# ExistentialRobotics/CORSAIR

Hardware: AMD Instinct MI355X
Metric: end-to-end queries/sec (embed+retrieve+register), Scan2CAD chair (higher is better)
Workload: dtype f32 sparse conv + embedding / f64 RANSAC, k-NN, Chamfer, top-k / f16 MFMA bounds and shortlists (survivors recounted in f64)

## Files before the change

### corsair_amd/csrc/ransac.hip

```cpp
#include <math.h>

#include <algorithm>
#include <atomic>
#include <vector>

#include "common.h"
#include "horn.h"

namespace cs {

using f32x16 = __attribute__((ext_vector_type(16))) float;
using f32x2 = __attribute__((ext_vector_type(2))) float;

struct RansacProb {
  int64_t off;
  int32_t m;
  int32_t est_k;
  int32_t best_cnt;
  int32_t best_itr;
  unsigned long long best_err;
  int32_t done;
  int32_t iters;
  int32_t n_cand;
  int32_t chunk_max;
  double best_T[12];
};

__device__ __forceinline__ RansacProb prob_view(const RansacProb* probs, int p) {
  RansacProb v = {};
  v.off = probs[p].off;
  v.m = probs[p].m;
  v.est_k = __atomic_load_n(&probs[p].est_k, __ATOMIC_RELAXED);
  v.done = __atomic_load_n(&probs[p].done, __ATOMIC_RELAXED);
  return v;
}

__host__ __device__ static inline uint32_t rng_index(uint64_t seed, uint64_t itr, uint64_t j,
                                                     uint32_t m) {
  return (uint32_t)(((rng_u64(seed, itr, j) >> 32) * (uint64_t)m) >> 32);
}

__global__ void k_ransac_pack(const float* __restrict__ src, const float* __restrict__ tgt,
                              int64_t n, float* __restrict__ pk, float4* __restrict__ pair32) {
  int64_t i = blockIdx.x * (int64_t)blockDim.x + threadIdx.x;
  if (i >= n) return;
  pair32[2 * i + 0] = make_float4(src[3 * i + 0], src[3 * i + 1], src[3 * i + 2], tgt[3 * i + 0]);
  pair32[2 * i + 1] = make_float4(tgt[3 * i + 1], tgt[3 * i + 2], 0.f, 0.f);
  pk[0 * n + i] = src[3 * i + 0];
  pk[1 * n + i] = src[3 * i + 1];
  pk[2 * n + i] = src[3 * i + 2];
  pk[3 * n + i] = tgt[3 * i + 0];
  pk[4 * n + i] = tgt[3 * i + 1];
  pk[5 * n + i] = tgt[3 * i + 2];
}

constexpr int XCD_SLOTS = 64;
struct XcdTab {
  int32_t v[8 * XCD_SLOTS];
};
__device__ __forceinline__ int xcd_problem(const int32_t* __restrict__ xcd_ptr, const XcdTab& tab, int i) {
  return xcd_ptr ? xcd_ptr[i] : tab.v[i];
}

__device__ __forceinline__ void pf_emit_row(const RansacProb& pr, int p, int h, int bmax, const double (&R)[3][3], double (&t)[3],
                                            const unsigned* __restrict__ stat, const double* __restrict__ sums, double thr2,
                                            double tcap, _Float16* __restrict__ A16, float* __restrict__ c_h);

template <int RN>
__global__ __launch_bounds__(256) void k_ransac_hyp(const RansacProb* probs,
                                                    const float4* __restrict__ pair32, int it0,
                                                    int bcount, int bmax, int ransac_n,
                                                    uint64_t seed,
                                                    const int32_t* __restrict__ xcd_prob, const XcdTab xcd_tab,
                                                    int slots, int tiles, int force_jacobi,
                                                    double* __restrict__ hyp,
                                                    const unsigned* __restrict__ pf_stat, const double* __restrict__ pf_sums,
                                                    double thr2, double tcap, _Float16* __restrict__ A16,
                                                    float* __restrict__ c_h, int32_t* __restrict__ cnt_zero) {
  const int xcd = blockIdx.x & 7;
  const int item = blockIdx.x >> 3;
  const int slot = item / tiles;
  const int p = xcd_problem(xcd_prob, xcd_tab, xcd * slots + slot);
  if (p < 0) return;
  const int h = (item - slot * tiles) * blockDim.x + threadIdx.x;
  if (h >= bcount) return;
  if (cnt_zero) cnt_zero[(int64_t)p * bmax + h] = 0;
  const RansacProb pr = prob_view(probs, p);
  const int itr = it0 + h;
  if (pr.done || itr >= pr.est_k) return;
  const uint32_t m = (uint32_t)pr.m;
  double cs_[3] = {0, 0, 0}, ct_[3] = {0, 0, 0};
  double S[3][3] = {{0, 0, 0}, {0, 0, 0}, {0, 0, 0}};
  if (RN > 0) {
    float4 pa[RN > 0 ? RN : 1];
    float2 pb[RN > 0 ? RN : 1];
#pragma unroll
    for (int j = 0; j < RN; ++j) {
      const int64_t i = pr.off + rng_index(seed, (uint64_t)itr, (uint64_t)j, m);
      const float4 a = pair32[2 * i], b = pair32[2 * i + 1];
      pa[j] = a;
      pb[j] = make_float2(b.x, b.y);
      cs_[0] += (double)a.x;
      cs_[1] += (double)a.y;
      cs_[2] += (double)a.z;
      ct_[0] += (double)a.w;
      ct_[1] += (double)b.x;
      ct_[2] += (double)b.y;
    }
    const double dn = (double)RN;
#pragma unroll
    for (int a = 0; a < 3; ++a) {
      cs_[a] = cs_[a] / dn;
      ct_[a] = ct_[a] / dn;
    }
#pragma unroll
    for (int j = 0; j < RN; ++j) {
      const double ds[3] = {(double)pa[j].x - cs_[0], (double)pa[j].y - cs_[1], (double)pa[j].z - cs_[2]};
      const double dt[3] = {(double)pa[j].w - ct_[0], (double)pb[j].x - ct_[1], (double)pb[j].y - ct_[2]};
#pragma unroll
      for (int a = 0; a < 3; ++a)
#pragma unroll
        for (int b = 0; b < 3; ++b) S[a][b] = fma(ds[a], dt[b], S[a][b]);
    }
  } else {
    for (int j = 0; j < ransac_n; ++j) {
      const int64_t i = pr.off + rng_index(seed, (uint64_t)itr, (uint64_t)j, m);
      const float4 a = pair32[2 * i], b = pair32[2 * i + 1];
      cs_[0] += (double)a.x;
      cs_[1] += (double)a.y;
      cs_[2] += (double)a.z;
      ct_[0] += (double)a.w;
      ct_[1] += (double)b.x;
      ct_[2] += (double)b.y;
    }
    const double dn = (double)ransac_n;
#pragma unroll
    for (int a = 0; a < 3; ++a) {
      cs_[a] = cs_[a] / dn;
      ct_[a] = ct_[a] / dn;
    }
    for (int j = 0; j < ransac_n; ++j) {
      const int64_t i = pr.off + rng_index(seed, (uint64_t)itr, (uint64_t)j, m);
      const float4 a = pair32[2 * i], b = pair32[2 * i + 1];
      const double ds[3] = {(double)a.x - cs_[0], (double)a.y - cs_[1], (double)a.z - cs_[2]};
      const double dt[3] = {(double)a.w - ct_[0], (double)b.x - ct_[1], (double)b.y - ct_[2]};
#pragma unroll
      for (int a = 0; a < 3; ++a)
#pragma unroll
        for (int b = 0; b < 3; ++b) S[a][b] = fma(ds[a], dt[b], S[a][b]);
    }
  }
  double N[4][4], V[4][4];
  N[0][0] = S[0][0] + S[1][1] + S[2][2];
  N[0][1] = S[1][2] - S[2][1];
  N[0][2] = S[2][0] - S[0][2];
  N[0][3] = S[0][1] - S[1][0];
  N[1][1] = S[0][0] - S[1][1] - S[2][2];
  N[1][2] = S[0][1] + S[1][0];
  N[1][3] = S[2][0] + S[0][2];
  N[2][2] = -S[0][0] + S[1][1] - S[2][2];
  N[2][3] = S[1][2] + S[2][1];
  N[3][3] = -S[0][0] - S[1][1] + S[2][2];
  N[1][0] = N[0][1];
  N[2][0] = N[0][2];
  N[3][0] = N[0][3];
  N[2][1] = N[1][2];
  N[3][1] = N[1][3];
  N[3][2] = N[2][3];
  double qv[4];
  if (force_jacobi || !horn_qcp(S, N, qv)) {
    jacobi4(N, V);
    double best = N[0][0];
    qv[0] = V[0][0]; qv[1] = V[1][0]; qv[2] = V[2][0]; qv[3] = V[3][0];
#pragma unroll
    for (int c = 1; c < 4; ++c) {
      if (N[c][c] > best) {
        best = N[c][c];
        qv[0] = V[0][c];
        qv[1] = V[1][c];
        qv[2] = V[2][c];
        qv[3] = V[3][c];
      }
    }
  }
  double qw = qv[0], qx = qv[1], qy = qv[2], qz = qv[3];
  const double qn = sqrt(qw * qw + qx * qx + qy * qy + qz * qz);
  qw = qw / qn;
  qx = qx / qn;
  qy = qy / qn;
  qz = qz / qn;
  double R[3][3];
  R[0][0] = 1.0 - 2.0 * (qy * qy + qz * qz);
  R[0][1] = 2.0 * (qx * qy - qw * qz);
// ... 107 lines not shown
    else
      atomicAdd(&res_cnt[(int64_t)p * bmax + hsel], cnt);
  }
}

template <bool LIST, int HPW = RC_HYP>
__global__ __launch_bounds__(256) void k_ransac_count(const RansacProb* __restrict__ probs,
                                                      const float* __restrict__ pk, int64_t total,
                                                      const double* __restrict__ hyp, int it0,
                                                      int bcount, int bmax, int splits, double thr2,
                                                      int32_t* __restrict__ res_cnt,
                                                      const int32_t* __restrict__ hlist,
                                                      const int32_t* __restrict__ n_surv) {
  __shared__ __attribute__((aligned(16))) double lds[2][RC_CHUNK][6];
  const int p = blockIdx.y;
  const int tile0 = blockIdx.x / splits;
  const int split = blockIdx.x - tile0 * splits;
  if (LIST) {
    const int nlist = n_surv[p];
    const int tstride = gridDim.x / splits;
    for (int tile = tile0; tile * RC_HYP < nlist; tile += tstride) {
      ransac_count_tile<LIST, HPW>(lds, p, tile, split, probs, pk, total, hyp, it0, bcount, bmax, splits, thr2,
                                   res_cnt, hlist, n_surv);
      __syncthreads();
    }
  } else {
    ransac_count_tile<LIST, HPW>(lds, p, tile0, split, probs, pk, total, hyp, it0, bcount, bmax, splits, thr2,
                                 res_cnt, hlist, n_surv);
  }
}

using f16x8 = __attribute__((ext_vector_type(8))) _Float16;
constexpr int PF_K = 16;
constexpr int PF_PITCH = 40;
constexpr int PF_PITCH1 = 24;
__host__ __device__ constexpr int pf_pitch(int nm) { return nm == 2 ? PF_PITCH : PF_PITCH1; }
constexpr int PF_ROWS = 192;
constexpr int PF_NG = 2;
constexpr int PF_HYP = 4 * 32 * PF_NG;
constexpr int PF_STAT = 17;
constexpr float PF_SMAX = 128.0f;

__device__ __forceinline__ _Float16 f16_of(double v) { return (_Float16)(float)v; }

__device__ __forceinline__ void split16(double v, _Float16* hi, _Float16* lo) {
  const _Float16 h = f16_of(v);
  *hi = h;
  *lo = f16_of(v - (double)h);
}

__host__ __device__ static inline int64_t pf_padded(int64_t m) { return (m + PF_ROWS - 1) / PF_ROWS * PF_ROWS; }

__global__ __launch_bounds__(256) void k_ransac_pair_sums(const RansacProb* __restrict__ probs, const float* __restrict__ src,
                                                          const float* __restrict__ tgt, double* __restrict__ sums) {
  __shared__ double red[4][6];
  const RansacProb pr = probs[blockIdx.x];
  double a[6] = {0, 0, 0, 0, 0, 0};
  for (int j = threadIdx.x; j < pr.m; j += 256) {
    const int64_t i = pr.off + j;
#pragma unroll
    for (int c = 0; c < 3; ++c) {
      a[c] += (double)src[3 * i + c];
      a[3 + c] += (double)tgt[3 * i + c];
    }
  }
#pragma unroll
  for (int c = 0; c < 6; ++c) {
#pragma unroll
    for (int off = 32; off >= 1; off >>= 1) a[c] += __shfl_xor(a[c], off);
    if ((threadIdx.x & 63) == 0) red[threadIdx.x >> 6][c] = a[c];
  }
  __syncthreads();
  if (threadIdx.x < 6) {
    const double sum = (red[0][threadIdx.x] + red[1][threadIdx.x]) + (red[2][threadIdx.x] + red[3][threadIdx.x]);
    const double v = sum / (double)(pr.m > 0 ? pr.m : 1);
    sums[blockIdx.x * 6 + threadIdx.x] = (v == v && fabs(v) < 1.0e30) ? v : 0.0;
  }
}
__device__ __forceinline__ void pf_centre(const double* __restrict__ sums, int p, int m, double (&mu)[6]) {
  (void)m;
#pragma unroll
  for (int c = 0; c < 6; ++c) mu[c] = sums[p * 6 + c];
}

template <int NM>
__global__ __launch_bounds__(256) void k_ransac_pack16(const RansacProb* __restrict__ probs,
                                                       const int64_t* __restrict__ off16,
                                                       const float* __restrict__ src,
                                                       const float* __restrict__ tgt,
                                                       const double* __restrict__ sums,
                                                       _Float16* __restrict__ B16,
                                                       unsigned* __restrict__ stat) {
  __shared__ float red[4][PF_STAT];
  const RansacProb pr = probs[blockIdx.y];
  double mu[6];
  pf_centre(sums, blockIdx.y, pr.m, mu);
  const int mpad = (int)pf_padded(pr.m);
  float mx[PF_STAT];
#pragma unroll
  for (int k = 0; k < PF_STAT; ++k) mx[k] = 0.f;
  for (int j = blockIdx.x * blockDim.x + threadIdx.x; j < mpad; j += gridDim.x * blockDim.x) {
    constexpr int NV = pf_pitch(NM) / 8;
    union {
      _Float16 h[PF_PITCH];
      uint4 v[5];
    } row;
#pragma unroll
    for (int k = 0; k < 5; ++k) row.v[k] = make_uint4(0u, 0u, 0u, 0u);
    if (j < pr.m) {
      const int64_t i = pr.off + j;
      const double sx = src[3 * i] - mu[0], sy = src[3 * i + 1] - mu[1], sz = src[3 * i + 2] - mu[2];
      const double qx = tgt[3 * i] - mu[3], qy = tgt[3 * i + 1] - mu[4], qz = tgt[3 * i + 2] - mu[5];
      const double ss = sx * sx + sy * sy + sz * sz, qq = qx * qx + qy * qy + qz * qz;
      double b[16];
      b[0] = ss + qq;
      b[1] = sx; b[2] = sy; b[3] = sz;
      b[4] = qx * sx; b[5] = qx * sy; b[6] = qx * sz;
      b[7] = qy * sx; b[8] = qy * sy; b[9] = qy * sz;
      b[10] = qz * sx; b[11] = qz * sy; b[12] = qz * sz;
      b[13] = qx; b[14] = qy; b[15] = qz;
      float mag = 1.0000002f * (float)sqrt(fmax(ss, qq));
      const bool ok = mag <= PF_SMAX;
      if (!(mag == mag)) mag = INFINITY;
#pragma unroll
      for (int k = 0; k < 16; ++k) {
        _Float16 hi = (_Float16)0.0f, lo = (_Float16)0.0f;
        if (ok) {
          split16(b[k], &hi, &lo);
          mx[1 + k] = fmaxf(mx[1 + k], __double2float_ru(fabs(b[k])));
        }
        row.h[k] = hi;
        if (NM == 2) row.h[16 + k] = lo;
      }
      mx[0] = fmaxf(mx[0], mag);
    } else {
      row.h[0] = (_Float16)60000.0f;
    }
    uint4* dst = reinterpret_cast<uint4*>(B16 + (off16[blockIdx.y] + j) * pf_pitch(NM));
#pragma unroll
    for (int k = 0; k < NV; ++k) dst[k] = row.v[k];
  }
#pragma unroll
  for (int k = 0; k < PF_STAT; ++k) {
#pragma unroll
    for (int off = 32; off >= 1; off >>= 1) mx[k] = fmaxf(mx[k], __shfl_xor(mx[k], off));
    if ((threadIdx.x & 63) == 0) red[threadIdx.x >> 6][k] = mx[k];
  }
  __syncthreads();
  if (threadIdx.x < PF_STAT) {
    const int k = threadIdx.x;
    const float m = fmaxf(fmaxf(red[0][k], red[1][k]), fmaxf(red[2][k], red[3][k]));
    if (m > 0.f) atomicMax(&stat[blockIdx.y * PF_STAT + k], __float_as_uint(m));
  }
}

__global__ __launch_bounds__(256) void k_ransac_pack16_b0(const RansacProb* __restrict__ probs,
                                                          const int64_t* __restrict__ off16,
                                                          const float* __restrict__ src, const float* __restrict__ tgt,
                                                          const double* __restrict__ sums,
                                                          const unsigned* __restrict__ stat, double tcap,
                                                          _Float16* __restrict__ B16) {
  const RansacProb pr = probs[blockIdx.y];
  double mu[6];
  pf_centre(sums, blockIdx.y, pr.m, mu);
  const double smax = (double)__uint_as_float(stat[blockIdx.y * PF_STAT]);
  if (!(smax <= (double)PF_SMAX)) return;
  const double beta = smax * smax;
  const double a_rot = 2.002 * (1.0 + 0x1p-11), a_t = 2.0 * tcap * smax * 1.0005 * (1.0 + 0x1p-11);
  for (int j = blockIdx.x * blockDim.x + threadIdx.x; j < pr.m; j += gridDim.x * blockDim.x) {
    const int64_t i = pr.off + j;
    const double sx = src[3 * i] - mu[0], sy = src[3 * i + 1] - mu[1], sz = src[3 * i + 2] - mu[2];
    const double qx = tgt[3 * i] - mu[3], qy = tgt[3 * i + 1] - mu[4], qz = tgt[3 * i + 2] - mu[5];
    const double ss = sx * sx + sy * sy + sz * sz, qq = qx * qx + qy * qy + qz * qz;
    const double b[16] = {ss + qq, sx, sy, sz, qx * sx, qx * sy, qx * sz, qy * sx, qy * sy, qy * sz,
                          qz * sx, qz * sy, qz * sz, qx, qy, qz};
    double e_t = 0.0, e_rot = 0.0;
#pragma unroll
    for (int k = 1; k < 16; ++k) {
      const double lo = fabs(b[k] - (double)f16_of(b[k]));
      if (k >= 4 && k <= 12) e_rot += lo; else e_t += lo;
    }
    const double ep = (1.0 + 0x1p-10) * (a_rot * e_rot + a_t * e_t);
    const double v = (b[0] - beta) - ep - 0x1p-40 * (fabs(b[0]) + beta + ep);
    _Float16 h = f16_of(v);
    if ((double)h > v) {
      unsigned short u = __builtin_bit_cast(unsigned short, h);
      u = (u & 0x8000u) ? (unsigned short)(u + 1) : (u == 0 ? (unsigned short)0x8001u : (unsigned short)(u - 1));
      h = __builtin_bit_cast(_Float16, u);
    }
    B16[(off16[blockIdx.y] + j) * PF_PITCH1] = h;
  }
}

__device__ __forceinline__ void pf_emit_row(const RansacProb& pr, int p, int h, int bmax, const double (&R)[3][3], double (&t)[3],
                                            const unsigned* __restrict__ stat, const double* __restrict__ sums, double thr2,
                                            double tcap, _Float16* __restrict__ A16, float* __restrict__ c_h) {
  {
    double mu[6];
    pf_centre(sums, p, pr.m, mu);
#pragma unroll
    for (int a = 0; a < 3; ++a) t[a] = t[a] + (R[a][0] * mu[0] + R[a][1] * mu[1] + R[a][2] * mu[2]) - mu[3 + a];
  }
  const double smax = (double)__uint_as_float(stat[p * PF_STAT]);
  const double tt = t[0] * t[0] + t[1] * t[1] + t[2] * t[2];
  const double tn = sqrt(tt);
  double a[16];
  a[0] = 1.0;
#pragma unroll
  for (int b = 0; b < 3; ++b) a[1 + b] = 2.0 * (R[0][b] * t[0] + R[1][b] * t[1] + R[2][b] * t[2]);
#pragma unroll
  for (int x = 0; x < 3; ++x)
#pragma unroll
    for (int b = 0; b < 3; ++b) a[4 + 3 * x + b] = -2.0 * R[x][b];
#pragma unroll
  for (int x = 0; x < 3; ++x) a[13 + x] = -2.0 * t[x];
  double dev = 0.0;
#pragma unroll
  for (int x = 0; x < 3; ++x)
#pragma unroll
    for (int y = 0; y < 3; ++y) {
      const double e = R[0][x] * R[0][y] + R[1][x] * R[1][y] + R[2][x] * R[2][y] - (x == y ? 1.0 : 0.0);
      dev = fmax(dev, fabs(e));
    }
  bool usable = smax <= (double)PF_SMAX && tn <= 4.0 * (double)PF_SMAX && dev < 1.0e-3;
  if (tcap > 0.0) usable = usable && tn <= tcap * smax;
  usable = usable && thr2 < 3.0e4;
  const double beta = tcap > 0.0 ? smax * smax : 0.0;
#pragma unroll
  for (int k = 0; k < 16; ++k) usable = usable && fabs(a[k]) < 6.0e4;
  union {
    _Float16 h[PF_K];
    uint4 v[2];
  } row;
  double drop = 0.0;
#pragma unroll
  for (int k = 0; k < 16; ++k) {
    const _Float16 hi = usable ? f16_of(a[k]) : (_Float16)0.0f;
    row.h[k] = hi;
    if (usable) drop += fabs(a[k] - (double)hi) * (double)__uint_as_float(stat[p * PF_STAT + 1 + k]);
  }
  uint4* dst = reinterpret_cast<uint4*>(A16 + ((int64_t)p * bmax + h) * PF_K);
  dst[0] = row.v[0];
  dst[1] = row.v[1];
// ... 655 lines not shown
struct Options {
  bool prefilter;
  bool check;
  int pf_nm;
  bool stage2;
  int first_chunk;
  int force_jacobi;
  bool overlap;
  int trace_it0;
  const char* trace_file;
};
Options read_options() {
  const char* pf = getenv("CS_RANSAC_PREFILTER");
  const char* ck = getenv("CS_RANSAC_CHECK");
  const char* k = getenv("CS_RANSAC_PF_K");
  const char* s2 = getenv("CS_RANSAC_STAGE2");
  const char* first = getenv("CS_RANSAC_FIRST");
  const char* jac = getenv("CS_RANSAC_JACOBI");
  const char* ov = getenv("CS_RANSAC_OVERLAP");
  const char* tr = getenv("CS_PF_TRACE");
  const char* trf = getenv("CS_PF_TRACE_FILE");
  Options o;
  o.prefilter = !(pf && pf[0] == '0');
  o.check = ck && ck[0] == '1';
  o.pf_nm = (k && atoi(k) == 32) ? 2 : 1;
  o.stage2 = !(s2 && s2[0] == '0');
  o.first_chunk = ((std::min(std::max(first ? atoi(first) : 64, 64), BMAX) + 63) / 64) * 64;
  o.force_jacobi = jac && atoi(jac) != 0;
  o.overlap = !(ov && ov[0] == '0');
  o.trace_it0 = tr ? atoi(tr) : -1;
  o.trace_file = trf ? trf : "/tmp/pf_trace.bin";
  return o;
}

struct Scratch {
  int n_prob = 0;
  size_t st_probs = 0, st_surv = 0, st_cnt = 0, st_bytes = 0;
  PoolBuf<char> state;
  char* h_state = nullptr;
  PoolBuf<float> pk;
  PoolBuf<float4> pair32;
  PoolBuf<double> hyp;
  PoolBuf<int32_t> res_cnt, cand;
  PoolBuf<unsigned long long> cand_err;
  PoolBuf<int64_t> off16;
  PoolBuf<_Float16> B16, A16;
  PoolBuf<float> c_h;
  PoolBuf<int32_t> cnt_up, hlist;
  PoolBuf<unsigned> pf_stat;
  PoolBuf<double> pf_sums;
  PoolBuf<_Float16> B32, A16s;
  PoolBuf<float> c_hs;
  PoolBuf<int32_t> cnt2;
  PoolBuf<unsigned> pf_stat2;
  PoolBuf<int32_t> exact_dbg;
  PoolBuf<unsigned long long> chk_stats;
  PoolBuf<int32_t> xcd_buf;
  PoolBuf<unsigned long long> trace;
  size_t trace_cap = 1;

  bool alloc(int n, int64_t tot1, int64_t rows16, int pf_nm, bool pf, bool stage2, bool check, bool tracing) {
    n_prob = n;
    st_probs = sizeof(RansacProb) * (size_t)n;
    st_surv = ((sizeof(int32_t) * (size_t)n + 7) / 8) * 8;
    st_cnt = st_surv + 8;
    st_bytes = st_probs + 2 * st_cnt;
    h_state = pinned_scratch(st_bytes);
    const size_t nb = (size_t)n * BMAX, ns2 = (size_t)n * PF_S2_CAP;
    if (tracing) trace_cap = (size_t)8 * n * 64 * 16 * 16;
    return h_state && state.alloc(st_bytes) && pk.alloc((size_t)tot1 * 6) && pair32.alloc((size_t)tot1 * 2) &&
           hyp.alloc(2 * nb * 12) && res_cnt.alloc(nb) && cand.alloc(nb) && cand_err.alloc(nb) && off16.alloc(n + 1) &&
           B16.alloc(pf ? (size_t)rows16 * pf_pitch(pf_nm) : 8) && A16.alloc(pf ? 2 * nb * PF_K : 8) &&
           c_h.alloc(pf ? 2 * nb : 1) && cnt_up.alloc(pf ? 2 * nb : 1) && hlist.alloc(pf ? nb : 1) &&
           pf_stat.alloc((size_t)n * PF_STAT) && pf_sums.alloc((size_t)n * 6) &&
           B32.alloc(stage2 ? (size_t)rows16 * PF_PITCH : 8) && A16s.alloc(stage2 ? ns2 * PF_K : 8) &&
           c_hs.alloc(stage2 ? ns2 : 1) && cnt2.alloc(stage2 ? ns2 : 1) && pf_stat2.alloc((size_t)n * PF_STAT) &&
           exact_dbg.alloc(check ? nb : 1) && chk_stats.alloc(4) && xcd_buf.alloc((size_t)16 * n) && trace.alloc(trace_cap);
  }
  RansacProb* probs() const { return reinterpret_cast<RansacProb*>(state.p); }
  int32_t* nsurv(int par) const { return reinterpret_cast<int32_t*>(state.p + st_probs + par * st_cnt); }
  int* nactive(int par) const { return reinterpret_cast<int*>(state.p + st_probs + par * st_cnt + st_surv); }
  const int32_t* h_nsurv(int par) const { return reinterpret_cast<const int32_t*>(h_state + st_probs + par * st_cnt); }
  int h_nactive(int par) const { return *reinterpret_cast<const int*>(h_state + st_probs + par * st_cnt + st_surv); }
  double* hyp_of(int par) const { return hyp.p + (size_t)par * n_prob * 12 * BMAX; }
  _Float16* A16_of(int par) const { return A16.p + (size_t)par * n_prob * BMAX * PF_K; }
  float* c_h_of(int par) const { return c_h.p + (size_t)par * n_prob * BMAX; }
  int32_t* cnt_up_of(int par) const { return cnt_up.p + (size_t)par * n_prob * BMAX; }
  int32_t* xcd_of(int par) const { return xcd_buf.p + (size_t)par * 8 * n_prob; }
};

struct Event {
  hipEvent_t e = nullptr;
  ~Event() {
    if (e) (void)hipEventDestroy(e);
  }
};
struct SideDrain {
  hipStream_t st = nullptr;
  bool clean = false;
  ~SideDrain() {
    if (st && !clean) (void)hipStreamSynchronize(st);
  }
};

struct Front {
  int it0 = 0, b = 0, par = 0;
  bool pf = false, on_side = false;
  XcdTab xtab;
  const int32_t* xcd_prob = nullptr;
  int pslots = 1;
};

struct RansacCall {
  int n_prob = 0, ransac_n = 0, max_iter = 0, m_max = 0;
  uint64_t seed = 0;
  int64_t total = 0, tot1 = 1;
  double thr2 = 0.0, scale = 0.0, log_1mc = 0.0, tcap = 0.0;
  Options opt;
  bool pf_alloc = false, stage2 = false, check = false;
  std::vector<RansacProb> hp;
  std::vector<int64_t> h_off16;
  std::vector<int32_t> h_xcd[2];
  Scratch sc;
  Event round_done, front_done[2], hyp_done[2];
  hipStream_t s = nullptr, side = nullptr, side_hyp = nullptr;
  SideDrain side_drain, side_hyp_drain;
  int max_surv_prev = 1 << 30;
  unsigned long long tot_surv = 0, tot_eval = 0;
  size_t trace_n = 0;
// ... 18 lines not shown
  int back_half(const Front& cur);
  int count_chunk(const Front& cur, double eval_pairs);
  int count_survivors(const Front& cur, bool* err_known);
  bool read_back(const Front& cur);
  int finish(float* d_T, int32_t* d_inliers, double* d_rmse, int32_t* d_iters);
};

int RansacCall::init(const int64_t* h_off, int n, double max_corr, int rn, int iters, double confidence, uint64_t sd,
                     hipStream_t st) {
  n_prob = n;
  ransac_n = rn;
  max_iter = iters;
  seed = sd;
  s = st;
  total = h_off[n_prob] - h_off[0];
  tot1 = total ? total : 1;
  hp.resize(n_prob);
  h_off16.assign(n_prob + 1, 0);
  for (int p = 0; p < n_prob; ++p) {
    int64_t m = h_off[p + 1] - h_off[p];
    CS_REQUIRE(m >= 0 && m < (1LL << 24), CS_ERR_INVALID,
               "cs_ransac_batch: bad segment %d (a problem holds fewer than 2^24 correspondences)", p);
    RansacProb& pr = hp[p];
    memset(&pr, 0, sizeof(pr));
    pr.off = h_off[p];
    pr.m = (int32_t)m;
    pr.est_k = max_iter;
    pr.best_itr = -1;
    pr.done = m < ransac_n ? 1 : 0;
    if (m > m_max) m_max = (int)m;
    h_off16[p + 1] = h_off16[p] + pf_padded(m);
  }
  thr2 = max_corr * max_corr;
  int ex = 0;
  (void)frexp(thr2, &ex);
  scale = ldexp(1.0, 38 - ex);
  log_1mc = log(1.0 - confidence);
  opt = read_options();
  pf_alloc = opt.prefilter && total > 0 && max_iter > opt.first_chunk;
  stage2 = pf_alloc && opt.pf_nm == 1 && opt.stage2;
  check = pf_alloc && opt.check;
  tcap = opt.pf_nm == 2 ? 0.0 : PF_TCAP;
  const bool ok = sc.alloc(n_prob, tot1, h_off16[n_prob] ? h_off16[n_prob] : 1, opt.pf_nm, pf_alloc, stage2, check,
                           opt.trace_it0 >= 0);
  CS_REQUIRE(ok, CS_ERR_HIP, "cs_ransac_batch: scratch allocation failed");
  return CS_OK;
}

int RansacCall::setup(const float* d_src, const float* d_tgt) {
  memset(sc.h_state, 0, sc.st_bytes);
  memcpy(sc.h_state, hp.data(), sc.st_probs);
  CS_HIP_CHECK(hipMemcpyAsync(sc.state.p, sc.h_state, sc.st_bytes, hipMemcpyHostToDevice, s));
  RansacProb* const d_probs = sc.probs();
  if (total > 0) {
    hipLaunchKernelGGL(k_ransac_pack, dim3((unsigned)ceil_div(total, 256)), dim3(256), 0, s,
                       d_src, d_tgt, total, sc.pk.p, sc.pair32.p);
    CS_LAUNCH_CHECK();
  }
  if (pf_alloc) {
    CS_HIP_CHECK(hipMemsetAsync(sc.pf_stat.p, 0, sizeof(unsigned) * n_prob * PF_STAT, s));
    CS_HIP_CHECK(hipMemsetAsync(sc.chk_stats.p, 0, sizeof(unsigned long long) * 4, s));
    int pblocks = (int)ceil_div(m_max > 0 ? m_max : 1, 256);
    if (pblocks > 64) pblocks = 64;
    const dim3 pgrid((unsigned)pblocks, (unsigned)n_prob);
    CS_HIP_CHECK(hipMemcpyAsync(sc.off16.p, h_off16.data(), sizeof(int64_t) * (n_prob + 1),
                                hipMemcpyHostToDevice, s));
    hipLaunchKernelGGL(k_ransac_pair_sums, dim3((unsigned)n_prob), dim3(256), 0, s, d_probs, d_src, d_tgt, sc.pf_sums.p);
    hipLaunchKernelGGL(opt.pf_nm == 2 ? k_ransac_pack16<2> : k_ransac_pack16<1>, pgrid, dim3(256), 0, s,
                       d_probs, sc.off16.p, d_src, d_tgt, sc.pf_sums.p, sc.B16.p, sc.pf_stat.p);
    if (opt.pf_nm == 1)
      hipLaunchKernelGGL(k_ransac_pack16_b0, pgrid, dim3(256), 0, s,
                         d_probs, sc.off16.p, d_src, d_tgt, sc.pf_sums.p, sc.pf_stat.p, tcap, sc.B16.p);
    if (stage2) {
      CS_HIP_CHECK(hipMemsetAsync(sc.pf_stat2.p, 0, sizeof(unsigned) * n_prob * PF_STAT, s));
      hipLaunchKernelGGL(k_ransac_pack16<2>, pgrid, dim3(256), 0, s,
                         d_probs, sc.off16.p, d_src, d_tgt, sc.pf_sums.p, sc.B32.p, sc.pf_stat2.p);
    }
    CS_LAUNCH_CHECK();
  }
  if (opt.trace_it0 >= 0) CS_HIP_CHECK(hipMemsetAsync(sc.trace.p, 0, sizeof(unsigned long long) * sc.trace_cap, s));
  return CS_OK;
}

int RansacCall::open_streams() {
  for (Event* ev : {&round_done, &front_done[0], &front_done[1], &hyp_done[0], &hyp_done[1]})
    CS_HIP_CHECK(hipEventCreateWithFlags(&ev->e, hipEventDisableTiming));
  side = opt.overlap ? side_stream() : nullptr;
  side_hyp = side ? side_stream(1) : nullptr;
  side_drain.st = side;
  side_hyp_drain.st = side_hyp;
  return CS_OK;
}

int RansacCall::place(int it0, int par, int* live) {
  std::vector<int> order;
  for (int p = 0; p < n_prob; ++p)
    if (!hp[p].done && hp[p].est_k > it0) order.push_back(p);
  *live = (int)order.size();
  std::sort(order.begin(), order.end(), [&](int a, int c) { return hp[a].m > hp[c].m; });
  std::vector<std::vector<int>> lists(8);
  int64_t load[8] = {0, 0, 0, 0, 0, 0, 0, 0};
  for (int p : order) {
    int best = 0;
    for (int x = 1; x < 8; ++x)
      if (load[x] < load[best]) best = x;
    lists[best].push_back(p);
    load[best] += pf_padded(hp[p].m);
  }
  int pslots = 1;
  for (int x = 0; x < 8; ++x) pslots = std::max(pslots, (int)lists[x].size());
  std::vector<int32_t>& tab = h_xcd[par];
  tab.assign((size_t)8 * pslots, -1);
  for (int x = 0; x < 8; ++x)
    for (size_t i = 0; i < lists[x].size(); ++i) tab[(size_t)x * pslots + i] = lists[x][i];
  return pslots;
}

Front RansacCall::enqueue_front(int it0, int par, hipStream_t st) {
  Front f;
  f.it0 = it0;
  f.b = chunk_of(it0);
  f.par = par;
  f.pf = prefiltered(it0);
  f.on_side = st != s;
  const int b = f.b;
  int live = 0;
  f.pslots = place(it0, par, &live);
  const int pslots = f.pslots;
  hipStream_t sh = (f.on_side && f.pf && side_hyp) ? side_hyp : st;
  if (pslots <= XCD_SLOTS) {
    memcpy(f.xtab.v, h_xcd[par].data(), sizeof(int32_t) * 8 * pslots);
  } else {
    (void)hipMemcpyAsync(sc.xcd_of(par), h_xcd[par].data(), sizeof(int32_t) * 8 * pslots, hipMemcpyHostToDevice, sh);
    f.xcd_prob = sc.xcd_of(par);
  }
  RansacProb* const d_probs = sc.probs();
  _Float16* A16_r = f.pf ? sc.A16_of(par) : nullptr;
  float* c_h_r = f.pf ? sc.c_h_of(par) : nullptr;
  int32_t* cnt_up_r = f.pf ? sc.cnt_up_of(par) : nullptr;
  const int ptiles = (b + PF_HYP - 1) / PF_HYP;
  int psplits = (int)((8 * 1024 + (int64_t)live * ptiles - 1) / std::max<int64_t>((int64_t)live * ptiles, 1));
  if (psplits < 1) psplits = 1;
  if (psplits > 16) psplits = 16;
  while (psplits > 1 && m_max / psplits < 8 * PF_ROWS) --psplits;
  {
    ProfScope prof("ransac_hyp", sh);
    const int htiles = (b + 255) / 256;
    int32_t* fz = psplits > 1 ? cnt_up_r : nullptr;
    const auto kernel = ransac_n == 10 ? k_ransac_hyp<10> : k_ransac_hyp<0>;
    hipLaunchKernelGGL(kernel, dim3((unsigned)(8 * pslots * htiles)), dim3(256), 0, sh, d_probs,
                       sc.pair32.p, it0, b, BMAX, ransac_n, seed, f.xcd_prob, f.xtab, pslots, htiles, opt.force_jacobi,
                       sc.hyp_of(par), sc.pf_stat.p, sc.pf_sums.p, thr2, tcap, A16_r, c_h_r, fz);
  }
  if (f.pf) {
    if (sh != st) {
      (void)hipEventRecord(hyp_done[par].e, sh);
      (void)hipStreamWaitEvent(st, hyp_done[par].e, 0);
    }
    ProfScope prof("ransac_pre", st);
    const unsigned nblk = (unsigned)(8 * pslots * ptiles * psplits);
    unsigned long long* tr = (opt.trace_it0 == it0) ? sc.trace.p : nullptr;
    const auto kernel = opt.pf_nm == 2 ? k_ransac_prefilter<2, false> : k_ransac_prefilter<1, true>;
    hipLaunchKernelGGL(kernel, dim3(nblk), dim3(256), 0, st, d_probs, sc.off16.p, sc.B16.p, A16_r, c_h_r, it0, b, BMAX,
                       psplits, f.xcd_prob, f.xtab, pslots, ptiles, cnt_up_r, tr, (const int32_t*)nullptr);
    if (tr) trace_n = (size_t)nblk * 16;
  }
  if (f.on_side) (void)hipEventRecord(front_done[par].e, st);
  return f;
}

int RansacCall::count_chunk(const Front& cur, double eval_pairs) {
  const int b = cur.b;
  const int hpw = b <= 64 ? 64 : RC_HYP;
  const int tiles = (b + hpw - 1) / hpw;
  const int splits = chunk_splits(tiles);
  if (splits > 1 || hpw != RC_HYP)
    CS_HIP_CHECK(hipMemset2DAsync(sc.res_cnt.p, sizeof(int32_t) * BMAX, 0, sizeof(int32_t) * b, n_prob, s));
  ProfScope prof("ransac_eval", s, 30.0 * eval_pairs);
  const dim3 grid((unsigned)(tiles * splits), (unsigned)n_prob);
  const auto kernel = hpw == 64 ? k_ransac_count<false, 64> : k_ransac_count<false, RC_HYP>;
  hipLaunchKernelGGL(kernel, grid, dim3(256), 0, s, sc.probs(), sc.pk.p, tot1, sc.hyp_of(cur.par), cur.it0, b, BMAX,
                     splits, thr2, sc.res_cnt.p, (const int32_t*)nullptr, (const int32_t*)nullptr);
  return CS_OK;
}

int RansacCall::count_survivors(const Front& cur, bool* err_known) {
  const int it0 = cur.it0, b = cur.b;
  RansacProb* const d_probs = sc.probs();
  const double* hyp_r = sc.hyp_of(cur.par);
  const int32_t* cnt_up_r = sc.cnt_up_of(cur.par);
  int32_t* const d_nsurv = sc.nsurv(cur.par);
  const int surv_cap = std::min(max_surv_prev, b);
  const bool few = max_surv_prev <= FEW_MAX || b <= FEW_MAX;
  const bool run_s2 = stage2 && few && surv_cap <= PF_S2_CAP;
  Stage2Rows s2rows{};
  if (run_s2) {
    s2rows.A16 = sc.A16_of(cur.par);
    s2rows.c_h = sc.c_h_of(cur.par);
    s2rows.stat = sc.pf_stat.p;
    s2rows.tcap = tcap;
    s2rows.A16s = sc.A16s.p;
    s2rows.c_hs = sc.c_hs.p;
    s2rows.cnt2 = sc.cnt2.p;
  }
// ... 193 lines not shown
```

Measured before the change: 1922.

## Fuse RANSAC setup packing kernels and replace centroid division with exact reciprocal

Merges the separate pack, stat memsets and stage-2 pack16 launches into one images kernel that writes pk, pair32 and the f16 image rows together. It also moves the stat and chk_stats zeroing into the pair-sums kernel, unrolls the pair-sums loads, and has pack16_b0 read pair32 instead of src/tgt. In the hypothesis kernel, centroid divisions become a reciprocal-multiply with an FMA correction, guarded by an exponent check, and the kernel gets a waves-per-EU hint plus an asm barrier to steer register use. The goal is fewer launches and less redundant memory traffic in setup, and cheaper f64 division. The cost is more complex kernels and the risk of changed occupancy or register spills.

```diff
diff --git a/corsair_amd/csrc/exact_div.h b/corsair_amd/csrc/exact_div.h
--- /dev/null
+++ b/corsair_amd/csrc/exact_div.h
@@ -0,0 +1,30 @@
+#pragma once
+#include <stdint.h>
+#include <string.h>
+
+#if defined(__HIPCC__)
+#define CS_XDIV_FN __host__ __device__ inline
+#else
+#include <math.h>
+#define CS_XDIV_FN static inline
+#endif
+
+namespace cs {
+
+CS_XDIV_FN double exact_div_recip(double n) {
+  return (n >= 1.0 && n <= 64.0 && n == (double)(int)n) ? 1.0 / n : 0.0;
+}
+
+CS_XDIV_FN bool exact_div_ok(double x) {
+  uint64_t b;
+  memcpy(&b, &x, sizeof(b));
+  return (uint32_t)((b >> 52) & 0x7ffu) - 123u <= 1800u;
+}
+
+CS_XDIV_FN double exact_div(double x, double n, double r) {
+  const double q0 = x * r;
+  const double e = fma(-q0, n, x);
+  return fma(e, r, q0);
+}
+
+}
diff --git a/corsair_amd/csrc/ransac.hip b/corsair_amd/csrc/ransac.hip
--- a/corsair_amd/csrc/ransac.hip
+++ b/corsair_amd/csrc/ransac.hip
@@ -5,6 +5,7 @@
 #include <vector>
 
 #include "common.h"
+#include "exact_div.h"
 #include "horn.h"
 
 namespace cs {
@@ -66,10 +67,30 @@
                                             const unsigned* __restrict__ stat, const double* __restrict__ sums, double thr2,
                                             double tcap, _Float16* __restrict__ A16, float* __restrict__ c_h);
 
+__device__ __forceinline__ void centroid_div(double (&cs_)[3], double (&ct_)[3], double dn, double inv_n) {
+  bool fast = inv_n != 0.0;
+#pragma unroll
+  for (int a = 0; a < 3; ++a) fast = fast && exact_div_ok(cs_[a]) && exact_div_ok(ct_[a]);
+  if (fast) {
+#pragma unroll
+    for (int a = 0; a < 3; ++a) {
+      cs_[a] = exact_div(cs_[a], dn, inv_n);
+      ct_[a] = exact_div(ct_[a], dn, inv_n);
+    }
+  } else {
+#pragma unroll
+    for (int a = 0; a < 3; ++a) {
+      cs_[a] = cs_[a] / dn;
+      ct_[a] = ct_[a] / dn;
+    }
+  }
+}
+
 template <int RN>
+__attribute__((amdgpu_waves_per_eu(5, 5)))
 __global__ __launch_bounds__(256) void k_ransac_hyp(const RansacProb* probs,
                                                     const float4* __restrict__ pair32, int it0,
-                                                    int bcount, int bmax, int ransac_n,
+                                                    int bcount, int bmax, int ransac_n, double inv_n,
                                                     uint64_t seed,
                                                     const int32_t* __restrict__ xcd_prob, const XcdTab xcd_tab,
                                                     int slots, int tiles, int force_jacobi,
@@ -92,35 +113,29 @@
   double cs_[3] = {0, 0, 0}, ct_[3] = {0, 0, 0};
   double S[3][3] = {{0, 0, 0}, {0, 0, 0}, {0, 0, 0}};
   if (RN > 0) {
-    float4 pa[RN > 0 ? RN : 1];
-    float2 pb[RN > 0 ? RN : 1];
+    float pa[RN > 0 ? RN : 1][6];
 #pragma unroll
     for (int j = 0; j < RN; ++j) {
       const int64_t i = pr.off + rng_index(seed, (uint64_t)itr, (uint64_t)j, m);
       const float4 a = pair32[2 * i], b = pair32[2 * i + 1];
-      pa[j] = a;
-      pb[j] = make_float2(b.x, b.y);
-      cs_[0] += (double)a.x;
-      cs_[1] += (double)a.y;
-      cs_[2] += (double)a.z;
-      ct_[0] += (double)a.w;
-      ct_[1] += (double)b.x;
-      ct_[2] += (double)b.y;
-    }
-    const double dn = (double)RN;
-#pragma unroll
-    for (int a = 0; a < 3; ++a) {
-      cs_[a] = cs_[a] / dn;
-      ct_[a] = ct_[a] / dn;
-    }
+      pa[j][0] = a.x; pa[j][1] = a.y; pa[j][2] = a.z; pa[j][3] = a.w; pa[j][4] = b.x; pa[j][5] = b.y;
+#pragma unroll
+      for (int c = 0; c < 3; ++c) {
+        cs_[c] += (double)pa[j][c];
+        ct_[c] += (double)pa[j][3 + c];
+      }
+    }
+    centroid_div(cs_, ct_, (double)RN, inv_n);
 #pragma unroll
     for (int j = 0; j < RN; ++j) {
-      const double ds[3] = {(double)pa[j].x - cs_[0], (double)pa[j].y - cs_[1], (double)pa[j].z - cs_[2]};
-      const double dt[3] = {(double)pa[j].w - ct_[0], (double)pb[j].x - ct_[1], (double)pb[j].y - ct_[2]};
-#pragma unroll
-      for (int a = 0; a < 3; ++a)
-#pragma unroll
-        for (int b = 0; b < 3; ++b) S[a][b] = fma(ds[a], dt[b], S[a][b]);
+#pragma unroll
+      for (int c = 0; c < 6; ++c) asm volatile("" : "+v"(pa[j][c]));
+      const double ds[3] = {(double)pa[j][0] - cs_[0], (double)pa[j][1] - cs_[1], (double)pa[j][2] - cs_[2]};
+      const double dt[3] = {(double)pa[j][3] - ct_[0], (double)pa[j][4] - ct_[1], (double)pa[j][5] - ct_[2]};
+#pragma unroll
+      for (int x = 0; x < 3; ++x)
+#pragma unroll
+        for (int y = 0; y < 3; ++y) S[x][y] = fma(ds[x], dt[y], S[x][y]);
     }
   } else {
     for (int j = 0; j < ransac_n; ++j) {
@@ -133,12 +148,7 @@
       ct_[1] += (double)b.x;
       ct_[2] += (double)b.y;
     }
-    const double dn = (double)ransac_n;
-#pragma unroll
-    for (int a = 0; a < 3; ++a) {
-      cs_[a] = cs_[a] / dn;
-      ct_[a] = ct_[a] / dn;
-    }
+    centroid_div(cs_, ct_, (double)ransac_n, inv_n);
     for (int j = 0; j < ransac_n; ++j) {
       const int64_t i = pr.off + rng_index(seed, (uint64_t)itr, (uint64_t)j, m);
       const float4 a = pair32[2 * i], b = pair32[2 * i + 1];
@@ -352,16 +362,32 @@
 __host__ __device__ static inline int64_t pf_padded(int64_t m) { return (m + PF_ROWS - 1) / PF_ROWS * PF_ROWS; }
 
 __global__ __launch_bounds__(256) void k_ransac_pair_sums(const RansacProb* __restrict__ probs, const float* __restrict__ src,
-                                                          const float* __restrict__ tgt, double* __restrict__ sums) {
+                                                          const float* __restrict__ tgt, double* __restrict__ sums,
+                                                          unsigned* __restrict__ stat, unsigned long long* __restrict__ chk_stats) {
   __shared__ double red[4][6];
   const RansacProb pr = probs[blockIdx.x];
+  if (threadIdx.x < PF_STAT) stat[blockIdx.x * PF_STAT + threadIdx.x] = 0u;
+  if (blockIdx.x == 0 && threadIdx.x < 4) chk_stats[threadIdx.x] = 0ull;
   double a[6] = {0, 0, 0, 0, 0, 0};
-  for (int j = threadIdx.x; j < pr.m; j += 256) {
-    const int64_t i = pr.off + j;
-#pragma unroll
-    for (int c = 0; c < 3; ++c) {
-      a[c] += (double)src[3 * i + c];
-      a[3 + c] += (double)tgt[3 * i + c];
+  constexpr int SUMS_U = 8;
+  for (int j0 = threadIdx.x; j0 < pr.m; j0 += 256 * SUMS_U) {
+    float v[SUMS_U][6];
+#pragma unroll
+    for (int u = 0; u < SUMS_U; ++u) {
+      const int j = j0 + 256 * u;
+      const int64_t i = pr.off + (j < pr.m ? j : j0);
+#pragma unroll
+      for (int c = 0; c < 3; ++c) {
+        v[u][c] = src[3 * i + c];
+        v[u][3 + c] = tgt[3 * i + c];
+      }
+    }
+#pragma unroll
+    for (int u = 0; u < SUMS_U; ++u) {
+      if (j0 + 256 * u < pr.m) {
+#pragma unroll
+        for (int c = 0; c < 6; ++c) a[c] += (double)v[u][c];
+      }
     }
   }
 #pragma unroll
@@ -383,14 +409,28 @@
   for (int c = 0; c < 6; ++c) mu[c] = sums[p * 6 + c];
 }
 
-template <int NM>
-__global__ __launch_bounds__(256) void k_ransac_pack16(const RansacProb* __restrict__ probs,
+__device__ __forceinline__ float pf_pair_row(float s0, float s1, float s2, float q0, float q1, float q2, const double (&mu)[6],
+                                             double (&b)[16]) {
+  const double sx = s0 - mu[0], sy = s1 - mu[1], sz = s2 - mu[2];
+  const double qx = q0 - mu[3], qy = q1 - mu[4], qz = q2 - mu[5];
+  const double ss = sx * sx + sy * sy + sz * sz, qq = qx * qx + qy * qy + qz * qz;
+  b[0] = ss + qq;
+  b[1] = sx; b[2] = sy; b[3] = sz;
+  b[4] = qx * sx; b[5] = qx * sy; b[6] = qx * sz;
+  b[7] = qy * sx; b[8] = qy * sy; b[9] = qy * sz;
+  b[10] = qz * sx; b[11] = qz * sy; b[12] = qz * sz;
+  b[13] = qx; b[14] = qy; b[15] = qz;
+  return 1.0000002f * (float)sqrt(fmax(ss, qq));
+}
+
+static_assert(PF_PITCH == 40 && PF_PITCH1 == 24, "k_ransac_images / k_ransac_pack16_b0 write 5 / 3 pieces of 16 B per row");
+__global__ __launch_bounds__(256) void k_ransac_images(const RansacProb* __restrict__ probs,
                                                        const int64_t* __restrict__ off16,
                                                        const float* __restrict__ src,
                                                        const float* __restrict__ tgt,
-                                                       const double* __restrict__ sums,
-                                                       _Float16* __restrict__ B16,
-                                                       unsigned* __restrict__ stat) {
+                                                       const double* __restrict__ sums, int64_t n,
+                                                       float* __restrict__ pk, float4* __restrict__ pair32,
+                                                       _Float16* __restrict__ B32, unsigned* __restrict__ stat) {
   __shared__ float red[4][PF_STAT];
   const RansacProb pr = probs[blockIdx.y];
   double mu[6];
@@ -400,7 +440,6 @@
 #pragma unroll
   for (int k = 0; k < PF_STAT; ++k) mx[k] = 0.f;
   for (int j = blockIdx.x * blockDim.x + threadIdx.x; j < mpad; j += gridDim.x * blockDim.x) {
-    constexpr int NV = pf_pitch(NM) / 8;
     union {
       _Float16 h[PF_PITCH];
       uint4 v[5];
@@ -409,17 +448,17 @@
     for (int k = 0; k < 5; ++k) row.v[k] = make_uint4(0u, 0u, 0u, 0u);
     if (j < pr.m) {
       const int64_t i = pr.off + j;
-      const double sx = src[3 * i] - mu[0], sy = src[3 * i + 1] - mu[1], sz = src[3 * i + 2] - mu[2];
-      const double qx = tgt[3 * i] - mu[3], qy = tgt[3 * i + 1] - mu[4], qz = tgt[3 * i + 2] - mu[5];
-      const double ss = sx * sx + sy * sy + sz * sz, qq = qx * qx + qy * qy + qz * qz;
+      const float fs[3] = {src[3 * i], src[3 * i + 1], src[3 * i + 2]};
+      const float fq[3] = {tgt[3 * i], tgt[3 * i + 1], tgt[3 * i + 2]};
+      pair32[2 * i + 0] = make_float4(fs[0], fs[1], fs[2], fq[0]);
+      pair32[2 * i + 1] = make_float4(fq[1], fq[2], 0.f, 0.f);
+#pragma unroll
+      for (int c = 0; c < 3; ++c) {
+        pk[c * n + i] = fs[c];
+        pk[(3 + c) * n + i] = fq[c];
+      }
       double b[16];
-      b[0] = ss + qq;
-      b[1] = sx; b[2] = sy; b[3] = sz;
-      b[4] = qx * sx; b[5] = qx * sy; b[6] = qx * sz;
-      b[7] = qy * sx; b[8] = qy * sy; b[9] = qy * sz;
-      b[10] = qz * sx; b[11] = qz * sy; b[12] = qz * sz;
-      b[13] = qx; b[14] = qy; b[15] = qz;
-      float mag = 1.0000002f * (float)sqrt(fmax(ss, qq));
+      float mag = pf_pair_row(fs[0], fs[1], fs[2], fq[0], fq[1], fq[2], mu, b);
       const bool ok = mag <= PF_SMAX;
       if (!(mag == mag)) mag = INFINITY;
 #pragma unroll
@@ -430,15 +469,18 @@
           mx[1 + k] = fmaxf(mx[1 + k], __double2float_ru(fabs(b[k])));
         }
         row.h[k] = hi;
-        if (NM == 2) row.h[16 + k] = lo;
+        row.h[16 + k] = lo;
       }
       mx[0] = fmaxf(mx[0], mag);
     } else {
       row.h[0] = (_Float16)60000.0f;
     }
-    uint4* dst = reinterpret_cast<uint4*>(B16 + (off16[blockIdx.y] + j) * pf_pitch(NM));
-#pragma unroll
-    for (int k = 0; k < NV; ++k) dst[k] = row.v[k];
+    const int64_t r = off16[blockIdx.y] + j;
+    if (B32) {
+      uint4* dst = reinterpret_cast<uint4*>(B32 + r * PF_PITCH);
+#pragma unroll
+      for (int k = 0; k < PF_PITCH / 8; ++k) dst[k] = row.v[k];
+    }
   }
 #pragma unroll
   for (int k = 0; k < PF_STAT; ++k) {
@@ -456,7 +498,7 @@
 
 __global__ __launch_bounds__(256) void k_ransac_pack16_b0(const RansacProb* __restrict__ probs,
                                                           const int64_t* __restrict__ off16,
-                                                          const float* __restrict__ src, const float* __restrict__ tgt,
+                                                          const float4* __restrict__ pair32,
                                                           const double* __restrict__ sums,
                                                           const unsigned* __restrict__ stat, double tcap,
                                                           _Float16* __restrict__ B16) {
@@ -464,31 +506,52 @@
   double mu[6];
   pf_centre(sums, blockIdx.y, pr.m, mu);
   const double smax = (double)__uint_as_float(stat[blockIdx.y * PF_STAT]);
-  if (!(smax <= (double)PF_SMAX)) return;
+  const bool bypass = !(smax <= (double)PF_SMAX);
   const double beta = smax * smax;
   const double a_rot = 2.002 * (1.0 + 0x1p-11), a_t = 2.0 * tcap * smax * 1.0005 * (1.0 + 0x1p-11);
-  for (int j = blockIdx.x * blockDim.x + threadIdx.x; j < pr.m; j += gridDim.x * blockDim.x) {
-    const int64_t i = pr.off + j;
-    const double sx = src[3 * i] - mu[0], sy = src[3 * i + 1] - mu[1], sz = src[3 * i + 2] - mu[2];
-    const double qx = tgt[3 * i] - mu[3], qy = tgt[3 * i + 1] - mu[4], qz = tgt[3 * i + 2] - mu[5];
-    const double ss = sx * sx + sy * sy + sz * sz, qq = qx * qx + qy * qy + qz * qz;
-    const double b[16] = {ss + qq, sx, sy, sz, qx * sx, qx * sy, qx * sz, qy * sx, qy * sy, qy * sz,
-                          qz * sx, qz * sy, qz * sz, qx, qy, qz};
-    double e_t = 0.0, e_rot = 0.0;
-#pragma unroll
-    for (int k = 1; k < 16; ++k) {
-      const double lo = fabs(b[k] - (double)f16_of(b[k]));
-      if (k >= 4 && k <= 12) e_rot += lo; else e_t += lo;
-    }
-    const double ep = (1.0 + 0x1p-10) * (a_rot * e_rot + a_t * e_t);
-    const double v = (b[0] - beta) - ep - 0x1p-40 * (fabs(b[0]) + beta + ep);
-    _Float16 h = f16_of(v);
-    if ((double)h > v) {
-      unsigned short u = __builtin_bit_cast(unsigned short, h);
-      u = (u & 0x8000u) ? (unsigned short)(u + 1) : (u == 0 ? (unsigned short)0x8001u : (unsigned short)(u - 1));
-      h = __builtin_bit_cast(_Float16, u);
-    }
-    B16[(off16[blockIdx.y] + j) * PF_PITCH1] = h;
+  const int mpad = (int)pf_padded(pr.m);
+  for (int j = blockIdx.x * blockDim.x + threadIdx.x; j < mpad; j += gridDim.x * blockDim.x) {
+    union {
+      _Float16 h[PF_PITCH1];
+      uint4 v[3];
+    } row;
+#pragma unroll
+    for (int k = 0; k < 3; ++k) row.v[k] = make_uint4(0u, 0u, 0u, 0u);
+    if (j < pr.m) {
+      const int64_t i = pr.off + j;
+      const float4 pa = pair32[2 * i], pb = pair32[2 * i + 1];
+      double b[16];
+      const float mag = pf_pair_row(pa.x, pa.y, pa.z, pa.w, pb.x, pb.y, mu, b);
+      if (bypass) {
+        if (mag <= PF_SMAX) {
+#pragma unroll
+          for (int k = 0; k < 16; ++k) row.h[k] = f16_of(b[k]);
+        }
+      } else {
+        double e_t = 0.0, e_rot = 0.0;
+#pragma unroll
+        for (int k = 1; k < 16; ++k) {
+          const _Float16 hi = f16_of(b[k]);
+          row.h[k] = hi;
+          const double lo = fabs(b[k] - (double)hi);
+          if (k >= 4 && k <= 12) e_rot += lo; else e_t += lo;
+        }
+        const double ep = (1.0 + 0x1p-10) * (a_rot * e_rot + a_t * e_t);
+        const double v = (b[0] - beta) - ep - 0x1p-40 * (fabs(b[0]) + beta + ep);
+        _Float16 h = f16_of(v);
+        if ((double)h > v) {
+          unsigned short u = __builtin_bit_cast(unsigned short, h);
+          u = (u & 0x8000u) ? (unsigned short)(u + 1) : (u == 0 ? (unsigned short)0x8001u : (unsigned short)(u - 1));
+          h = __builtin_bit_cast(_Float16, u);
+        }
+        row.h[0] = h;
+      }
+    } else {
+      row.h[0] = (_Float16)60000.0f;
+    }
+    uint4* dst = reinterpret_cast<uint4*>(B16 + (off16[blockIdx.y] + j) * PF_PITCH1);
+#pragma unroll
+    for (int k = 0; k < 3; ++k) dst[k] = row.v[k];
   }
 }
 
@@ -1250,7 +1313,6 @@
   PoolBuf<_Float16> B32, A16s;
   PoolBuf<float> c_hs;
   PoolBuf<int32_t> cnt2;
-  PoolBuf<unsigned> pf_stat2;
   PoolBuf<int32_t> exact_dbg;
   PoolBuf<unsigned long long> chk_stats;
   PoolBuf<int32_t> xcd_buf;
@@ -1272,7 +1334,7 @@
            c_h.alloc(pf ? 2 * nb : 1) && cnt_up.alloc(pf ? 2 * nb : 1) && hlist.alloc(pf ? nb : 1) &&
            pf_stat.alloc((size_t)n * PF_STAT) && pf_sums.alloc((size_t)n * 6) &&
            B32.alloc(stage2 ? (size_t)rows16 * PF_PITCH : 8) && A16s.alloc(stage2 ? ns2 * PF_K : 8) &&
-           c_hs.alloc(stage2 ? ns2 : 1) && cnt2.alloc(stage2 ? ns2 : 1) && pf_stat2.alloc((size_t)n * PF_STAT) &&
+           c_hs.alloc(stage2 ? ns2 : 1) && cnt2.alloc(stage2 ? ns2 : 1) &&
            exact_dbg.alloc(check ? nb : 1) && chk_stats.alloc(4) && xcd_buf.alloc((size_t)16 * n) && trace.alloc(trace_cap);
   }
   RansacProb* probs() const { return reinterpret_cast<RansacProb*>(state.p); }
@@ -1397,30 +1459,23 @@
   memcpy(sc.h_state, hp.data(), sc.st_probs);
   CS_HIP_CHECK(hipMemcpyAsync(sc.state.p, sc.h_state, sc.st_bytes, hipMemcpyHostToDevice, s));
   RansacProb* const d_probs = sc.probs();
-  if (total > 0) {
-    hipLaunchKernelGGL(k_ransac_pack, dim3((unsigned)ceil_div(total, 256)), dim3(256), 0, s,
-                       d_src, d_tgt, total, sc.pk.p, sc.pair32.p);
-    CS_LAUNCH_CHECK();
-  }
   if (pf_alloc) {
-    CS_HIP_CHECK(hipMemsetAsync(sc.pf_stat.p, 0, sizeof(unsigned) * n_prob * PF_STAT, s));
-    CS_HIP_CHECK(hipMemsetAsync(sc.chk_stats.p, 0, sizeof(unsigned long long) * 4, s));
     int pblocks = (int)ceil_div(m_max > 0 ? m_max : 1, 256);
     if (pblocks > 64) pblocks = 64;
     const dim3 pgrid((unsigned)pblocks, (unsigned)n_prob);
     CS_HIP_CHECK(hipMemcpyAsync(sc.off16.p, h_off16.data(), sizeof(int64_t) * (n_prob + 1),
                                 hipMemcpyHostToDevice, s));
-    hipLaunchKernelGGL(k_ransac_pair_sums, dim3((unsigned)n_prob), dim3(256), 0, s, d_probs, d_src, d_tgt, sc.pf_sums.p);
-    hipLaunchKernelGGL(opt.pf_nm == 2 ? k_ransac_pack16<2> : k_ransac_pack16<1>, pgrid, dim3(256), 0, s,
-                       d_probs, sc.off16.p, d_src, d_tgt, sc.pf_sums.p, sc.B16.p, sc.pf_stat.p);
+    hipLaunchKernelGGL(k_ransac_pair_sums, dim3((unsigned)n_prob), dim3(256), 0, s, d_probs, d_src, d_tgt, sc.pf_sums.p,
+                       sc.pf_stat.p, sc.chk_stats.p);
+    hipLaunchKernelGGL(k_ransac_images, pgrid, dim3(256), 0, s, d_probs, sc.off16.p, d_src, d_tgt, sc.pf_sums.p, total,
+                       sc.pk.p, sc.pair32.p, opt.pf_nm == 2 ? sc.B16.p : (stage2 ? sc.B32.p : nullptr), sc.pf_stat.p);
     if (opt.pf_nm == 1)
       hipLaunchKernelGGL(k_ransac_pack16_b0, pgrid, dim3(256), 0, s,
-                         d_probs, sc.off16.p, d_src, d_tgt, sc.pf_sums.p, sc.pf_stat.p, tcap, sc.B16.p);
-    if (stage2) {
-      CS_HIP_CHECK(hipMemsetAsync(sc.pf_stat2.p, 0, sizeof(unsigned) * n_prob * PF_STAT, s));
-      hipLaunchKernelGGL(k_ransac_pack16<2>, pgrid, dim3(256), 0, s,
-                         d_probs, sc.off16.p, d_src, d_tgt, sc.pf_sums.p, sc.B32.p, sc.pf_stat2.p);
-    }
+                         d_probs, sc.off16.p, sc.pair32.p, sc.pf_sums.p, sc.pf_stat.p, tcap, sc.B16.p);
+    CS_LAUNCH_CHECK();
+  } else if (total > 0) {
+    hipLaunchKernelGGL(k_ransac_pack, dim3((unsigned)ceil_div(total, 256)), dim3(256), 0, s,
+                       d_src, d_tgt, total, sc.pk.p, sc.pair32.p);
     CS_LAUNCH_CHECK();
   }
   if (opt.trace_it0 >= 0) CS_HIP_CHECK(hipMemsetAsync(sc.trace.p, 0, sizeof(unsigned long long) * sc.trace_cap, s));
@@ -1494,7 +1549,7 @@
     int32_t* fz = psplits > 1 ? cnt_up_r : nullptr;
     const auto kernel = ransac_n == 10 ? k_ransac_hyp<10> : k_ransac_hyp<0>;
     hipLaunchKernelGGL(kernel, dim3((unsigned)(8 * pslots * htiles)), dim3(256), 0, sh, d_probs,
-                       sc.pair32.p, it0, b, BMAX, ransac_n, seed, f.xcd_prob, f.xtab, pslots, htiles, opt.force_jacobi,
+                       sc.pair32.p, it0, b, BMAX, ransac_n, exact_div_recip((double)ransac_n), seed, f.xcd_prob, f.xtab, pslots, htiles, opt.force_jacobi,
                        sc.hyp_of(par), sc.pf_stat.p, sc.pf_sums.p, thr2, tcap, A16_r, c_h_r, fz);
   }
   if (f.pf) {
```

After: 2030 (median of 6 runs). 1.06x the previous value.
